# bevyengine/bevy

Measured on NVIDIA H100. Metric: entities/s propagate+cull+cluster @1M ents/256 lights, higher is better.
Workload: dtype f32

## Files before the change

bevy_b200/csrc/kernels.cu:

```cuda
#include <cstdint>
#include <cstdlib>
#include <cuda_runtime.h>

#include "device_types.cuh"
#include "kernels.cuh"

namespace b200vis {

struct Aff { float4 r0, r1, r2; };

__device__ __forceinline__ Aff affine_from_trs(float4 A, float4 q, float2 C) {
    const float sx = A.w, sy = C.x, sz = C.y;
    const float x2 = q.x + q.x, y2 = q.y + q.y, z2 = q.z + q.z;
    const float xx = q.x * x2, xy = q.x * y2, xz = q.x * z2;
    const float yy = q.y * y2, yz = q.y * z2, zz = q.z * z2;
    const float wx = q.w * x2, wy = q.w * y2, wz = q.w * z2;
    Aff a;
    a.r0 = make_float4((1.0f - (yy + zz)) * sx, (xy - wz) * sy, (xz + wy) * sz, A.x);
    a.r1 = make_float4((xy + wz) * sx, (1.0f - (xx + zz)) * sy, (yz - wx) * sz, A.y);
    a.r2 = make_float4((xz - wy) * sx, (yz + wx) * sy, (1.0f - (xx + yy)) * sz, A.z);
    return a;
}

__device__ __forceinline__ float4 affine_mul_row(float4 p, const Aff &l) {
// ... 321 lines not shown
__device__ __forceinline__ void mbar_wait_guarded(unsigned long long *bar, uint32_t parity) {
    uint32_t done = 0, spins = 0;
    while (true) {
        asm volatile("{\n.reg .pred p;\nmbarrier.try_wait.parity.shared::cta.b64 p, [%1], %2;\nselp.u32 %0, 1, 0, p;\n}\n"
                     : "=r"(done) : "r"(smem_u32(bar)), "r"(parity) : "memory");
        if (done) break;
        if (++spins > (1u << 24)) __trap();
    }
}
__device__ __forceinline__ void mbar_arrive_cta(unsigned long long *bar) {
    asm volatile("mbarrier.arrive.shared::cta.b64 _, [%0];" ::"r"(smem_u32(bar)) : "memory");
}
__device__ __forceinline__ void bulk_g2s(void *dst, const void *src, uint32_t bytes, unsigned long long *bar) {
    asm volatile("cp.async.bulk.shared::cluster.global.mbarrier::complete_tx::bytes [%0], [%1], %2, [%3];"
                 ::"r"(smem_u32(dst)), "l"(src), "r"(bytes), "r"(smem_u32(bar)) : "memory");
}
__device__ __forceinline__ void bulk_s2g(void *dst, const void *src, uint32_t bytes) {
    asm volatile("cp.async.bulk.global.shared::cta.bulk_group [%0], [%1], %2;" ::"l"(dst), "r"(smem_u32(src)), "r"(bytes) : "memory");
}

__device__ __forceinline__ void cp_async_16(void *dst, const void *src) {
    asm volatile("cp.async.cg.shared.global [%0], [%1], 16;" ::"r"(smem_u32(dst)), "l"(src) : "memory");
}
__device__ __forceinline__ void cp_async_8(void *dst, const void *src) {
    asm volatile("cp.async.ca.shared.global [%0], [%1], 8;" ::"r"(smem_u32(dst)), "l"(src) : "memory");
}
template <bool PROP, bool CULL>
__device__ __forceinline__ void issue_tile_loads(const Rows &R, const Tile &t, TileStage &S, unsigned long long *bar) {
    const uint32_t a = t.base & ~15u;
    const uint32_t cnt = ((t.base - a) + t.n_rows + 15u) & ~15u;
    uint32_t bytes = cnt * (48u + 2u);
    if (PROP) bytes += cnt * (40u + 4u);
    mbar_expect_tx(bar, bytes);
    bulk_g2s(S.gt0, R.gt0 + a, cnt * 16u, bar); bulk_g2s(S.gt1, R.gt1 + a, cnt * 16u, bar); bulk_g2s(S.gt2, R.gt2 + a, cnt * 16u, bar);
    bulk_g2s(S.flags, R.flags + a, cnt, bar); bulk_g2s(S.state, R.state + a, cnt, bar);
    if (PROP) {
        bulk_g2s(S.trsA, R.trsA + a, cnt * 16u, bar); bulk_g2s(S.trsB, R.trsB + a, cnt * 16u, bar);
        bulk_g2s(S.trsC, R.trsC + a, cnt * 8u, bar); bulk_g2s(S.topo, R.topo + a, cnt * 4u, bar);
    }
}

#ifdef B200VIS_TILE_TIMING
__device__ unsigned long long g_tile_timing[8192 * 16];
#define TT(slot) do { if (lr == 0 && blockIdx.x < 8192u) g_tile_timing[blockIdx.x * 16u + (slot)] = clock64(); } while (0)
#define TTW(slot) do { if (lr == 224u && blockIdx.x < 8192u) g_tile_timing[blockIdx.x * 16u + (slot)] = clock64(); } while (0)
__device__ unsigned long long g_tile_phase[8192 * 32];
#define TP_BEGIN() __shared__ unsigned long long tp_acc_[32]; unsigned long long tp_prev_ = clock64(); uint32_t tp_n_ = 0; \
    if (lr == 0) for (int k_ = 0; k_ < 32; ++k_) tp_acc_[k_] = 0ull
#define TP(ph) do { if (lr == 0) { const unsigned long long now_ = clock64(); \
    if ((ph) == 0) { ++tp_n_; tp_acc_[0] += 1ull; if (tp_n_ > 1u) tp_acc_[16] += 1ull; } \
    else { tp_acc_[(ph)] += now_ - tp_prev_; if (tp_n_ > 1u) tp_acc_[16 + (ph)] += now_ - tp_prev_; } \
    tp_prev_ = now_; } } while (0)
#define TP_END() do { if (lr == 0 && blockIdx.x < 8192u) for (int k_ = 0; k_ < 32; ++k_) g_tile_phase[blockIdx.x * 32u + k_] = tp_acc_[k_]; } while (0)
#else
#define TT(slot) do { } while (0)
#define TTW(slot) do { } while (0)
#define TP_BEGIN() do { } while (0)
#define TP(ph) do { } while (0)
#define TP_END() do { } while (0)
#endif
#define B200VIS_TILE_1B k_propagate_cull_tma
#define B200VIS_TILE_1B_EXT false
#include "tile_kernel_1b.cuh"
#undef B200VIS_TILE_1B
#undef B200VIS_TILE_1B_EXT
#define B200VIS_TILE_1B k_propagate_cull_tma_ext
#define B200VIS_TILE_1B_EXT true
#include "tile_kernel_1b.cuh"
#undef B200VIS_TILE_1B
#undef B200VIS_TILE_1B_EXT

template <bool WITH_TRS> struct __align__(128) LeanStage;
template <> struct __align__(128) LeanStage<true> {
    float4 gt0[kWin], gt1[kWin], gt2[kWin];
    uint32_t topo[kWin];
    uint8_t flags[kWin], state[kWin];
    float4 trsA[kWin], trsB[kWin];
    float2 trsC[kWin];
};
template <> struct __align__(128) LeanStage<false> {
    float4 gt0[kWin], gt1[kWin], gt2[kWin];
    uint32_t topo[kWin];
    uint8_t flags[kWin], state[kWin];
};
template <bool WITH_TRS>
struct LeanSmem {
    LeanStage<WITH_TRS> st[2];
    unsigned long long bar[2];
    Tile tdesc[3];
    uint32_t next_tile[2];
    float4 vplanes[kMaxViews * 5];
    float vlen[kMaxViews * 5];
    unsigned long long done[2];
    uint32_t anyflag[2];
    uint16_t parent[kTileRows];
    uint8_t pst[2][kTileRows];
    uint8_t dirty[kTileRows];
};
template <bool PROP, bool CULL, bool WITH_TRS>
__device__ __forceinline__ void issue_lean_loads(const Rows &R, const Tile &t, LeanStage<WITH_TRS> &S, unsigned long long *bar) {
    const uint32_t a = t.base & ~15u;
    const uint32_t cnt = ((t.base - a) + t.n_rows + 15u) & ~15u;
    uint32_t bytes = cnt * (48u + 2u);
    if (PROP) bytes += cnt * 4u;
    if (PROP && WITH_TRS) bytes += cnt * 40u;
    mbar_expect_tx(bar, bytes);
    bulk_g2s(S.gt0, R.gt0 + a, cnt * 16u, bar); bulk_g2s(S.gt1, R.gt1 + a, cnt * 16u, bar); bulk_g2s(S.gt2, R.gt2 + a, cnt * 16u, bar);
    bulk_g2s(S.flags, R.flags + a, cnt, bar); bulk_g2s(S.state, R.state + a, cnt, bar);
    if (PROP) bulk_g2s(S.topo, R.topo + a, cnt * 4u, bar);
    if constexpr (WITH_TRS) {
        if (PROP) {
            bulk_g2s(S.trsA, R.trsA + a, cnt * 16u, bar); bulk_g2s(S.trsB, R.trsB + a, cnt * 16u, bar);
// ... 1520 lines not shown
            uint32_t *cc = vb.chunk_count + ((size_t)parity * kMaxViews + v) * vb.chunks_stride;
            atomicOr(mask + (rnk >> 5), 1u << (rnk & 31u));
            atomicAdd(cc + ((rnk >> 5) / kChunkWords), 1u);
        }
    }
    if (SIMPLE || R.rank == nullptr) {
        if (lane < cvw.n_views && (cvw.on[lane] & 1u) && (!SIMPLE || (cvw.on[lane] & 4u))) {
            const uint32_t w0 = (row - lane) >> 5;
            if (w0 < vb.n_words) {
                vb.mask[(size_t)lane * vb.words_stride + w0] = my_ballot;
                if (my_ballot) atomicAdd(vb.chunk_count + ((size_t)parity * kMaxViews + lane) * vb.chunks_stride + (w0 / kChunkWords), __popc(my_ballot));
            }
        }
    }
    if (MERGE) {
        const bool merge = in_query && any && !(st8 & 1u);
        const uint32_t was = (st8 & S_VV_CHANGED) ? 1u : 0u;
        if (merge) R.state[row] = (uint8_t)((st8 & ~(S_VV | S_VV_CHANGED)) | 1u | (was << 1) | (was ? 0u : S_VV_CHANGED));
        const uint32_t up = __ballot_sync(0xFFFFFFFFu, merge && !was), down = __ballot_sync(0xFFFFFFFFu, merge && was);
        if (lane == 0 && up != down) atomicAdd(&stats->changed[parity][1], (uint32_t)(__popc(up) - __popc(down)));
        return;
    }
    uint32_t out = st8;
    bool vv_changed = false;
    if (in_query) {
        out = (st8 & ~(S_VV | S_VV_CHANGED)) | (any ? (1u | (prev << 1)) : 0u);
        vv_changed = (any ? 1u : 0u) != prev;
        if (vv_changed) out |= S_VV_CHANGED;
    } else {
        out = st8 & ~S_VV_CHANGED;
    }
    if (active && out != st8) R.state[row] = (uint8_t)out;
    if (R.light_snap != nullptr && (f & F_SPHERE_GT) && active) {
        const uint32_t ord = R.light_ord[row];
        if (ord < R.n_lights) R.light_snap[ord] = make_float4(g.r0.w, g.r1.w, g.r2.w, (out & 1u) ? 1.0f : 0.0f);
    }
    const uint32_t bv = __ballot_sync(0xFFFFFFFFu, vv_changed);
    if (lane == 0 && bv) atomicAdd(&stats->changed[parity][1], __popc(bv));
}

__global__ void k_mark_dirty_global(Rows R) {
    const uint32_t row = blockIdx.x * blockDim.x + threadIdx.x;
    if (row >= R.n || !(R.flags[row] & F_TCHANGED)) return;
    uint32_t c = row;
    while (true) {
        if (R.dirty[c]) break;
        R.dirty[c] = 1;
        const uint32_t p = R.parent[c];
        if (p >= R.n) break;
        c = p;
    }
}

__global__ void __launch_bounds__(kChunkWords)
k_expand_visible(VisibleBufs vb, DiffBufs db, const uint32_t *__restrict__ row_of_rank, const FrameConsts *__restrict__ fc,
                 DevStats *__restrict__ stats, uint32_t parity, uint32_t n_rows) {
    __shared__ uint32_t s_warp[32], s_diff[32];
    __shared__ uint32_t s_base, s_total;
    const uint32_t v = blockIdx.y, chunk = blockIdx.x, t = threadIdx.x;
    uint32_t *cc = vb.chunk_count + chunk_counter_index(parity, v) * vb.chunks_stride;
    const uint32_t zslot = (parity + 2u) % 3u;
    uint32_t *cc_next = vb.chunk_count + chunk_counter_index(zslot, v) * vb.chunks_stride;
    if (t == 0) cc_next[chunk] = 0;
    if (chunk == 0 && v == 0 && t < 2) stats->changed[zslot][t] = 0;
    if (v >= fc->n_views) {
        if (db.prev != nullptr && t == 0) db.chunk[(size_t)v * vb.chunks_stride + chunk] = 0;
        return;
    }
    if (!(fc->views[v].flags & 1u)) {
        if (db.prev != nullptr && t == 0) db.chunk[(size_t)v * vb.chunks_stride + chunk] = 0;
        return;
    }

    const uint32_t word = chunk * kChunkWords + t;
    uint32_t *mask = vb.mask + (size_t)v * vb.words_stride;
    uint32_t w = 0;
    if (word < vb.n_words) { w = mask[word]; if (w) mask[word] = 0; }
    const uint32_t c = __popc(w);
    if (db.prev != nullptr) {
        uint32_t a = 0, r = 0;
        if (word < vb.n_words) {
            uint32_t *pv = db.prev + (size_t)v * vb.words_stride + word;
            const uint32_t old = *pv;
            a = w & ~old; r = old & ~w;
            if (old != w) *pv = w;
            db.words[(size_t)v * vb.words_stride + word] = a;
            db.words[((size_t)gridDim.y + v) * vb.words_stride + word] = r;
        }
        uint32_t d = __popc(a) | (__popc(r) << 16);
#pragma unroll
        for (int o = 16; o > 0; o >>= 1) d += __shfl_xor_sync(0xFFFFFFFFu, d, o);
        if ((t & 31u) == 0) s_diff[t >> 5] = d;
    }
    uint32_t incl = c;
#pragma unroll
    for (int o = 1; o < 32; o <<= 1) { const uint32_t y = __shfl_up_sync(0xFFFFFFFFu, incl, o); if ((t & 31u) >= (uint32_t)o) incl += y; }
    if ((t & 31u) == 31u) s_warp[t >> 5] = incl;
    uint32_t part = 0, tot = 0;
    if (t < 32) {
        for (uint32_t i = t; i < vb.n_chunks; i += 32) { const uint32_t x = cc[i]; tot += x; if (i < chunk) part += x; }
#pragma unroll
        for (int o = 16; o > 0; o >>= 1) { part += __shfl_xor_sync(0xFFFFFFFFu, part, o); tot += __shfl_xor_sync(0xFFFFFFFFu, tot, o); }
        if (t == 0) { s_base = part; s_total = tot; }
    }
    __syncthreads();
    if (t < 32) {
        if (db.prev != nullptr) {
            uint32_t d = s_diff[t];
#pragma unroll
            for (int o = 16; o > 0; o >>= 1) d += __shfl_xor_sync(0xFFFFFFFFu, d, o);
            if (t == 0) db.chunk[(size_t)v * vb.chunks_stride + chunk] = d;
        }
        uint32_t x = s_warp[t];
#pragma unroll
        for (int o = 1; o < 32; o <<= 1) { const uint32_t y = __shfl_up_sync(0xFFFFFFFFu, x, o); if (t >= (uint32_t)o) x += y; }
        s_warp[t] = x;
    }
    __syncthreads();
    uint32_t pos = s_base + (incl - c) + ((t >> 5) ? s_warp[(t >> 5) - 1] : 0u);
    uint32_t *out = vb.lists + (size_t)v * vb.list_stride;
    uint8_t *out_cls = vb.classes ? vb.classes + (size_t)v * vb.list_stride : nullptr;
    while (w) {
        const uint32_t b = __ffs(w) - 1; w &= w - 1;
        const uint32_t rk = word * 32u + b;
        const uint32_t rw = row_of_rank ? row_of_rank[rk] : rk;
        if (out_cls) out_cls[pos] = vb.cls[rw];
        out[pos++] = rw;
    }
    if (chunk == 0 && t == 0) stats->visible_count[v] = s_total;
    (void)n_rows;
}

__global__ void __launch_bounds__(kChunkWords)
k_emit_visible_diff(VisibleBufs vb, DiffBufs db, const uint32_t *__restrict__ row_of_rank, const FrameConsts *__restrict__ fc) {
    __shared__ uint32_t s_warp[32];
    __shared__ uint32_t s_base[2], s_total[2];
    const uint32_t v = blockIdx.y, chunk = blockIdx.x, t = threadIdx.x;
    if (v >= fc->n_views || !(fc->views[v].flags & 1u)) {
        if (chunk == 0 && t < 2) db.count[v * 2 + t] = 0;
        return;
    }
    const uint32_t word = chunk * kChunkWords + t;
    uint32_t a = 0, r = 0;
    if (word < vb.n_words) {
        a = db.words[(size_t)v * vb.words_stride + word];
        r = db.words[((size_t)gridDim.y + v) * vb.words_stride + word];
    }
    const uint32_t c = __popc(a) | (__popc(r) << 16);
    uint32_t incl = c;
#pragma unroll
    for (int o = 1; o < 32; o <<= 1) { const uint32_t y = __shfl_up_sync(0xFFFFFFFFu, incl, o); if ((t & 31u) >= (uint32_t)o) incl += y; }
    if ((t & 31u) == 31u) s_warp[t >> 5] = incl;
    if (t < 32) {
        const uint32_t *cc = db.chunk + (size_t)v * vb.chunks_stride;
        uint32_t pa = 0, pr = 0, ta = 0, tr = 0;
        for (uint32_t i = t; i < vb.n_chunks; i += 32) {
            const uint32_t x = cc[i], xa = x & 0xFFFFu, xr = x >> 16;
            ta += xa; tr += xr;
            if (i < chunk) { pa += xa; pr += xr; }
        }
#pragma unroll
        for (int o = 16; o > 0; o >>= 1) {
            pa += __shfl_xor_sync(0xFFFFFFFFu, pa, o); pr += __shfl_xor_sync(0xFFFFFFFFu, pr, o);
            ta += __shfl_xor_sync(0xFFFFFFFFu, ta, o); tr += __shfl_xor_sync(0xFFFFFFFFu, tr, o);
        }
        if (t == 0) { s_base[0] = pa; s_base[1] = pr; s_total[0] = ta; s_total[1] = tr; }
    }
    __syncthreads();
    if (t < 32) {
        uint32_t x = s_warp[t];
#pragma unroll
        for (int o = 1; o < 32; o <<= 1) { const uint32_t y = __shfl_up_sync(0xFFFFFFFFu, x, o); if (t >= (uint32_t)o) x += y; }
        s_warp[t] = x;
    }
    __syncthreads();
    const uint32_t excl = (incl - c) + ((t >> 5) ? s_warp[(t >> 5) - 1] : 0u);
    uint32_t pos_a = s_base[0] + (excl & 0xFFFFu), pos_r = s_base[1] + (excl >> 16);
    uint32_t *out_a = db.lists + (size_t)v * vb.list_stride;
    uint32_t *out_r = db.lists + ((size_t)gridDim.y + v) * vb.list_stride;
    while (a) { const uint32_t b = __ffs(a) - 1; a &= a - 1; const uint32_t rk = word * 32u + b; out_a[pos_a++] = row_of_rank ? row_of_rank[rk] : rk; }
// ... 126 lines not shown
    return ((e[0] & w[0]) | (e[1] & w[1]) | (e[2] & w[2])) != 0ull;
}

template <bool EXT>
__global__ void __launch_bounds__(256)
k_cluster_assign(Rows R, Lights L, const FrameConsts *__restrict__ fc, ClusterBufs cb, DevStats *__restrict__ stats) {
    __shared__ float4 s_planes[kStagedPlanes];
    __shared__ float s_thr[kStagedPlanes];
    const uint32_t v = blockIdx.y;
    if (v >= fc->n_views) return;
    const DevClusterView &cv = fc->cviews[v];
    if (!cv.enabled) return;
    const uint32_t nx = cv.dims[0] + 1, ny_p = cv.dims[1] + 1, nz = cv.dims[2] + 1;
    const bool staged = nx + ny_p + nz <= kStagedPlanes;
    if (staged) {
        const float4 *gx = reinterpret_cast<const float4 *>(cb.blob + cv.x_off);
        const float4 *gy = reinterpret_cast<const float4 *>(cb.blob + cv.y_off);
        const float4 *gz = reinterpret_cast<const float4 *>(cb.blob + cv.z_off);
        for (uint32_t i = threadIdx.x; i < nx; i += 256) s_planes[i] = gx[i];
        for (uint32_t i = threadIdx.x; i < ny_p; i += 256) s_planes[nx + i] = gy[i];
        for (uint32_t i = threadIdx.x; i < nz; i += 256) s_planes[nx + ny_p + i] = gz[i];
        for (uint32_t i = threadIdx.x; i + 1 < cv.dims[2]; i += 256) s_thr[i] = cb.blob[cv.thr_off + i];
        __syncthreads();
    }
    const uint32_t li = blockIdx.x * 8u + (threadIdx.x >> 5), lane = threadIdx.x & 31u;
    if (li >= L.n) return;
    float px, py, pz;
    if (L.snap != nullptr) {
        const float4 sp = L.snap[li];
        if (sp.w == 0.0f) return;
        px = sp.x; py = sp.y; pz = sp.z;
    } else {
        const uint32_t row = L.row[li];
        if (!(R.state[row] & 1u)) return;
        px = R.gt0[row].w; py = R.gt1[row].w; pz = R.gt2[row].w;
    }
    const unsigned long long ll = L.layers ? L.layers[li] : 1ull;
    if (!(cv.layer_mask & ll) && !(EXT && light_layers_ext_intersect(L, fc, v, li))) return;
    const float range = L.range[li];
    ClusterTables tb;
    tb.thr = staged ? s_thr : cb.blob + cv.thr_off;
    tb.xp = staged ? s_planes : reinterpret_cast<const float4 *>(cb.blob + cv.x_off);
    tb.yp = staged ? s_planes + nx : reinterpret_cast<const float4 *>(cb.blob + cv.y_off);
    tb.zp = staged ? s_planes + nx + ny_p : reinterpret_cast<const float4 *>(cb.blob + cv.z_off);
    uint32_t *mask = cb.send + ((size_t)v * cb.words + (li >> 5)) * kMaxClusters;
    const uint32_t bit = 1u << (li & 31u);
    uint32_t count = 0;
    float this_far = 0.0f;
    if (!assign_one_light(cv, tb, px, py, pz, range, lane, this_far, count, [&](uint32_t ci) { atomicOr(mask + ci, bit); })) return;
    if (lane == 0 && this_far > 0.0f) atomicMax(cb.send + (cb.slab_words - cb.trailer) + v, __float_as_uint(this_far));
    (void)count; (void)stats;
}

constexpr uint32_t kFusedThreads = 1024;
__device__ __forceinline__ uint32_t cluster_ctarank() { uint32_t r; asm volatile("mov.u32 %0, %%cluster_ctarank;" : "=r"(r)); return r; }
__device__ __forceinline__ uint32_t cluster_nctarank() { uint32_t r; asm volatile("mov.u32 %0, %%cluster_nctarank;" : "=r"(r)); return r; }
__device__ __forceinline__ void cluster_sync_all() {
    asm volatile("barrier.cluster.arrive.release.aligned;\n\tbarrier.cluster.wait.acquire.aligned;" ::: "memory");
}
__device__ __forceinline__ uint32_t dsmem_addr(const void *p, uint32_t cta) {
    uint32_t a = (uint32_t)__cvta_generic_to_shared(p), r;
    asm volatile("mapa.shared::cluster.u32 %0, %1, %2;" : "=r"(r) : "r"(a), "r"(cta));
    return r;
}
__device__ __forceinline__ void dsmem_or(uint32_t addr, uint32_t v) {
    asm volatile("red.relaxed.cluster.shared::cluster.or.b32 [%0], %1;" ::"r"(addr), "r"(v) : "memory");
}
__device__ __forceinline__ uint32_t dsmem_ld(uint32_t addr) {
    uint32_t v; asm volatile("ld.shared::cluster.u32 %0, [%1];" : "=r"(v) : "r"(addr) : "memory"); return v;
}

__device__ __forceinline__ void st_release_sys(uint32_t *p, uint32_t v) {
    asm volatile("st.release.sys.global.u32 [%0], %1;" ::"l"(p), "r"(v) : "memory");
}
__device__ __forceinline__ uint32_t ld_acquire_sys(const uint32_t *p) {
    uint32_t v;
    asm volatile("ld.acquire.sys.global.u32 %0, [%1];" : "=r"(v) : "l"(p) : "memory");
    return v;
}
template <bool EXT>
__global__ void __launch_bounds__(kFusedThreads)
k_cluster_fused(Rows R, Lights L, const FrameConsts *__restrict__ fc, ClusterBufs cb, DevStats *__restrict__ stats) {
    extern __shared__ __align__(16) uint8_t smem_fused[];
    __shared__ float4 s_planes[kStagedPlanes];
    __shared__ float s_thr[kStagedPlanes];
    __shared__ uint32_t s_warp[32];
    __shared__ uint32_t s_total, s_far, s_base, s_farmax;
    const uint32_t v = blockIdx.y, t = threadIdx.x, lane = t & 31u, warp = t >> 5;
    const uint32_t rank = cluster_ctarank(), nrank = cluster_nctarank();
    uint32_t *offsets = cb.offsets + (size_t)v * (kMaxClusters + 1);
    if (v >= fc->n_views) return;
    const DevClusterView &cv = fc->cviews[v];
    if (!cv.enabled) {
        if (rank == 0 && t == 0) { offsets[0] = 0; stats->cl_overflow[v] = 0; stats->cl_index_count[v] = 0; stats->cl_farthest_bits[v] = 0; }
        return;
    }
    if (cb.p2p && L.per_rank) {
        if (t < cb.world) {
            const uint32_t *flag = cb.peer_flags[cb.rank] + cb.xparity * cb.world + t;
            uint32_t spins = 0;
            while ((int32_t)(ld_acquire_sys(flag) - cb.stamp) < 0) {
                __nanosleep(64);
                if (++spins > (1u << 22)) { stats->cl_overflow[v] = 2u; break; }
            }
        }
        __syncthreads();
    }
    const uint32_t nc = cv.n_clusters, per = (nc + nrank - 1) / nrank, words = (L.n + 31u) / 32u;
    uint32_t *s_mask = reinterpret_cast<uint32_t *>(smem_fused);
    for (uint32_t i = t; i < words * per; i += kFusedThreads) s_mask[i] = 0;
    if (t == 0) { s_total = 0; s_far = 0; }
    const uint32_t nx = cv.dims[0] + 1, ny_p = cv.dims[1] + 1, nz = cv.dims[2] + 1;
    const bool staged = nx + ny_p + nz <= kStagedPlanes;
    if (staged) {
        const float4 *gx = reinterpret_cast<const float4 *>(cb.blob + cv.x_off);
        const float4 *gy = reinterpret_cast<const float4 *>(cb.blob + cv.y_off);
        const float4 *gz = reinterpret_cast<const float4 *>(cb.blob + cv.z_off);
        for (uint32_t i = t; i < nx; i += kFusedThreads) s_planes[i] = gx[i];
        for (uint32_t i = t; i < ny_p; i += kFusedThreads) s_planes[nx + i] = gy[i];
        for (uint32_t i = t; i < nz; i += kFusedThreads) s_planes[nx + ny_p + i] = gz[i];
        for (uint32_t i = t; i + 1 < cv.dims[2]; i += kFusedThreads) s_thr[i] = cb.blob[cv.thr_off + i];
    }
    cluster_sync_all();
    ClusterTables tb;
    tb.thr = staged ? s_thr : cb.blob + cv.thr_off;
    tb.xp = staged ? s_planes : reinterpret_cast<const float4 *>(cb.blob + cv.x_off);
    tb.yp = staged ? s_planes + nx : reinterpret_cast<const float4 *>(cb.blob + cv.y_off);
    tb.zp = staged ? s_planes + nx + ny_p : reinterpret_cast<const float4 *>(cb.blob + cv.z_off);
    for (uint32_t li = rank + nrank * warp; li < L.n; li += nrank * (kFusedThreads / 32)) {
        float px, py, pz;
        if (L.snap != nullptr || L.per_rank) {
            const float4 sp = light_snap_of(L, li);
            if (sp.w == 0.0f) continue;
            px = sp.x; py = sp.y; pz = sp.z;
        } else {
            const uint32_t row = L.row[li];
            if (!(R.state[row] & 1u)) continue;
            px = R.gt0[row].w; py = R.gt1[row].w; pz = R.gt2[row].w;
        }
        const unsigned long long ll = light_layers_of(L, li);
        if (!(cv.layer_mask & ll) && !(EXT && light_layers_ext_intersect(L, fc, v, li))) continue;
        const uint32_t bit = 1u << (li & 31u), wbase = (li >> 5) * per;
        uint32_t count = 0;
        float this_far = 0.0f;
        const bool in = assign_one_light(cv, tb, px, py, pz, light_range_of(L, li), lane, this_far, count, [&](uint32_t ci) {
            const uint32_t owner = ci / per;
            dsmem_or(dsmem_addr(&s_mask[wbase + (ci - owner * per)], owner), bit);
        });
        if (in && lane == 0 && this_far > 0.0f) atomicMax(&s_far, __float_as_uint(this_far));
    }
    cluster_sync_all();
    const uint32_t first = rank * per, c = first + t;
    uint32_t cnt = 0;
    if (t < per && c < nc)
        for (uint32_t w = 0; w < words; ++w) cnt += __popc(s_mask[w * per + t]);
    uint32_t incl = cnt;
#pragma unroll
    for (int o = 1; o < 32; o <<= 1) { const uint32_t y = __shfl_up_sync(0xFFFFFFFFu, incl, o); if (lane >= (uint32_t)o) incl += y; }
    if (lane == 31u) s_warp[warp] = incl;
    __syncthreads();
    if (t < 32) {
        uint32_t x = s_warp[t];
#pragma unroll
        for (int o = 1; o < 32; o <<= 1) { const uint32_t y = __shfl_up_sync(0xFFFFFFFFu, x, o); if (t >= (uint32_t)o) x += y; }
        s_warp[t] = x;
        if (t == 31) s_total = x;
    }
    cluster_sync_all();
    if (t < 32) {
        uint32_t tot_r = 0, far_r = 0;
        if (t < nrank) { tot_r = dsmem_ld(dsmem_addr(&s_total, t)); far_r = dsmem_ld(dsmem_addr(&s_far, t)); }
        uint32_t b = (t < rank) ? tot_r : 0u, fm = far_r;
#pragma unroll
        for (int o = 16; o > 0; o >>= 1) {
            b += __shfl_xor_sync(0xFFFFFFFFu, b, o);
            fm = max(fm, __shfl_xor_sync(0xFFFFFFFFu, fm, o));
        }
        if (t == 0) { s_base = b; s_farmax = fm; }
    }
    asm volatile("barrier.cluster.arrive.release.aligned;" ::: "memory");
    __syncthreads();
    const uint32_t base = s_base;
    uint32_t pos = base + (incl - cnt) + (warp ? s_warp[warp - 1] : 0u);
    uint32_t *indices = cb.indices + (size_t)v * cb.index_cap;
    if (t < per && c < nc) {
        offsets[c] = pos;
        for (uint32_t w = 0; w < words; ++w) {
            uint32_t m = s_mask[w * per + t];
            while (m) {
                const uint32_t b = __ffs(m) - 1; m &= m - 1;
                if (pos < cb.index_cap) indices[pos] = w * 32u + b;
                ++pos;
            }
        }
        if (c == nc - 1) {
            offsets[nc] = pos;
            stats->cl_overflow[v] = pos > cb.index_cap ? 1u : 0u;
            stats->cl_index_count[v] = pos;
        }
    }
    if (rank == 0 && t == 0) stats->cl_farthest_bits[v] = s_farmax;
    asm volatile("barrier.cluster.wait.acquire.aligned;" ::: "memory");
}

constexpr uint32_t kListBlocks = kMaxClusters / 1024;

__global__ void __launch_bounds__(256)
k_slab_push(const FrameConsts *__restrict__ fc, ClusterBufs cb, uint32_t *__restrict__ done) {
    const uint32_t v = blockIdx.y;
    const size_t slab_words = cb.slab_words;
    if (blockIdx.x == 0 && threadIdx.x < cb.world && v < cb.trailer) {
        const size_t tr = ((size_t)cb.xparity * cb.world + cb.rank) * slab_words + (slab_words - cb.trailer) + v;
        cb.peer[threadIdx.x][tr] = cb.send[(slab_words - cb.trailer) + v];
    }
    if (v < fc->n_views && fc->cviews[v].enabled) {
// ... 1488 lines not shown
    }
    if (tile_kernel_is_tma()) {
#define B200VIS_LAUNCH_TMA(P, C, S) do { if (tile_kernel_choice() == 4) launch_tma<P, C, S, 1>(st, R, tiles, n_tiles, cvw, vb, stats, static_opt, parity, ticket, ticket_base); \
                                         else if (tile_kernel_choice() == 5 && lean_ctas_per_sm() == 4 && (P) && (C) && named_levels_only && lean_pipe()) launch_tma<P, C, S, 7>(st, R, tiles, n_tiles, cvw, vb, stats, static_opt, parity, ticket, ticket_base); \
                                         else if (tile_kernel_choice() == 5 && lean_ctas_per_sm() == 4) launch_tma<P, C, S, 4>(st, R, tiles, n_tiles, cvw, vb, stats, static_opt, parity, ticket, ticket_base); \
                                         else if (tile_kernel_choice() == 5 && lean_ctas_per_sm() == 6) launch_tma<P, C, S, 6>(st, R, tiles, n_tiles, cvw, vb, stats, static_opt, parity, ticket, ticket_base); \
                                         else if (tile_kernel_choice() == 5) launch_tma<P, C, S, 5>(st, R, tiles, n_tiles, cvw, vb, stats, static_opt, parity, ticket, ticket_base); \
                                         else launch_tma<P, C, S, 0>(st, R, tiles, n_tiles, cvw, vb, stats, static_opt, parity, ticket, ticket_base, rev); } while (0)
        if (prop && cull) { if (simple) B200VIS_LAUNCH_TMA(true, true, true); else B200VIS_LAUNCH_TMA(true, true, false); }
        else if (prop) B200VIS_LAUNCH_TMA(true, false, true);
        else if (cull) { if (simple) B200VIS_LAUNCH_TMA(false, true, true); else B200VIS_LAUNCH_TMA(false, true, false); }
#undef B200VIS_LAUNCH_TMA
        return;
    }
#define B200VIS_LAUNCH(P, C, S) ++g_launches, k_propagate_cull<P, C, S><<<n_tiles, kTileRows, 0, st>>>(R, tiles, cvw, vb, stats, static_opt, parity)
    if (prop && cull) { if (simple) B200VIS_LAUNCH(true, true, true); else B200VIS_LAUNCH(true, true, false); }
    else if (prop) B200VIS_LAUNCH(true, false, true);
    else if (cull) { if (simple) B200VIS_LAUNCH(false, true, true); else B200VIS_LAUNCH(false, true, false); }
#undef B200VIS_LAUNCH
}
void launch_propagate_cull_ext(cudaStream_t st, const Rows &R, const Tile *tiles, uint32_t n_tiles, const CullViews &cvw,
                               const VisibleBufs &vb, DevStats *stats, uint32_t stages, uint32_t static_opt, uint32_t parity,
                               uint32_t *ticket, uint32_t *ticket_base, uint32_t rev) {
    if (n_tiles == 0 || !(stages & 1u)) return;
    const bool simple = R.layers == nullptr && R.layers_ext == nullptr && R.range == nullptr && R.rank == nullptr;
    if (!(stages & 2u)) launch_tma<true, false, true, 8>(st, R, tiles, n_tiles, cvw, vb, stats, static_opt, parity, ticket, ticket_base, rev);
    else if (simple) launch_tma<true, true, true, 8>(st, R, tiles, n_tiles, cvw, vb, stats, static_opt, parity, ticket, ticket_base, rev);
    else launch_tma<true, true, false, 8>(st, R, tiles, n_tiles, cvw, vb, stats, static_opt, parity, ticket, ticket_base, rev);
}
bool tile_kernel_is_default() { return tile_kernel_choice() == 1; }
void launch_cull(cudaStream_t st, const Rows &R, const CullViews &cvw, const VisibleBufs &vb, DevStats *stats, uint32_t parity,
                 uint32_t rev) {
    if (!R.n) return;
    const bool simple = R.layers == nullptr && R.layers_ext == nullptr && R.range == nullptr && R.rank == nullptr;
    if (simple) { ++g_launches; k_cull<true, false><<<cdiv(R.n, 256), 256, 0, st>>>(R, cvw, vb, stats, parity, rev); }
    else { ++g_launches; k_cull<false, false><<<cdiv(R.n, 256), 256, 0, st>>>(R, cvw, vb, stats, parity, rev); }
}
void launch_cull_group(cudaStream_t st, const Rows &R, const CullViews &cvw, const VisibleBufs &vb, DevStats *stats, uint32_t parity,
                       uint32_t view_base, uint32_t rev) {
    if (!R.n) return;
    VisibleBufs g = vb;
    g.mask = vb.mask + (size_t)view_base * vb.words_stride;
    g.chunk_count = vb.chunk_count + chunk_counter_index(0, view_base) * vb.chunks_stride;
    const bool simple = R.layers == nullptr && R.layers_ext == nullptr && R.range == nullptr && R.rank == nullptr;
    if (simple) { ++g_launches; k_cull<true, true><<<cdiv(R.n, 256), 256, 0, st>>>(R, cvw, g, stats, parity, rev); }
    else { ++g_launches; k_cull<false, true><<<cdiv(R.n, 256), 256, 0, st>>>(R, cvw, g, stats, parity, rev); }
}
void launch_mark_dirty_global(cudaStream_t st, const Rows &R) {
    if (R.n) { ++g_launches; k_mark_dirty_global<<<cdiv(R.n, 256), 256, 0, st>>>(R); }
}
void launch_expand_visible(cudaStream_t st, const VisibleBufs &vb, const DiffBufs &db, const uint32_t *row_of_rank, const FrameConsts *fc,
                           DevStats *stats, uint32_t parity, uint32_t n_rows, uint32_t max_views) {
    if (vb.n_chunks == 0) return;
    ++g_launches; k_expand_visible<<<dim3(vb.n_chunks, max_views), kChunkWords, 0, st>>>(vb, db, row_of_rank, fc, stats, parity, n_rows);
    if (db.prev != nullptr) { ++g_launches; k_emit_visible_diff<<<dim3(vb.n_chunks, max_views), kChunkWords, 0, st>>>(vb, db, row_of_rank, fc); }
}
void launch_view_diff(cudaStream_t st, const VisibleBufs &vb, const ViewDiff &vd, const ViewSlots &vs, const uint32_t *row_of_rank,
                      const FrameConsts *fc, uint32_t parity, uint32_t slotted_views) {
    if (vb.n_chunks == 0 || slotted_views == 0) return;
    ++g_launches; k_view_diff<<<dim3(vb.n_chunks, slotted_views), kChunkWords, 0, st>>>(vb, vd, vs, row_of_rank, fc, parity);
}
void launch_emit_view_diff(cudaStream_t st, const VisibleBufs &vb, const ViewDiff &vd, const ViewSlots &vs, uint32_t n_views,
                           uint32_t slotted_views) {
    const uint32_t n_chunks = slotted_views ? vb.n_chunks : 0u;
    ++g_launches; k_view_diff_offsets<<<1, 1024, 0, st>>>(vd, vs, n_views * 8u, n_chunks, vb.chunks_stride);
    if (n_chunks == 0) return;
    ++g_launches; k_emit_view_diff<<<dim3(n_chunks, slotted_views), kChunkWords, 0, st>>>(vd, vs, vb.n_words, vb.words_stride, vb.chunks_stride);
}
void launch_publish_visible_diff(cudaStream_t st, const VisibleBufs &vb, const DiffBufs &db, uint32_t *host_rows, uint32_t host_stride,
                                 uint32_t *host_counts, uint32_t n_views, uint32_t max_views) {
    if (!n_views || db.prev == nullptr) return;
    ++g_launches; k_publish_visible_diff<<<dim3(32, n_views, 2), 256, 0, st>>>(db, vb.list_stride, host_rows, host_stride, host_counts, n_views, max_views);
}
void launch_cluster_assign(cudaStream_t st, const Rows &R, const Lights &L, const FrameConsts *fc, const ClusterBufs &cb,
                           DevStats *stats, uint32_t max_views) {
    if (L.n == 0) return;
    ++g_launches;
    if (L.layers_ext != nullptr) k_cluster_assign<true><<<dim3(cdiv(L.n, 8), max_views), 256, 0, st>>>(R, L, fc, cb, stats);
    else k_cluster_assign<false><<<dim3(cdiv(L.n, 8), max_views), 256, 0, st>>>(R, L, fc, cb, stats);
}
bool cluster_fused_fits(uint32_t n_lights) {
    const char *e = getenv("B200VIS_CLUSTER_KERNEL");
    if (e && e[0] == 's') return false;
    const size_t words = (n_lights + 31u) / 32u;
    return words * (kMaxClusters / 16) * 4 <= 200u * 1024u;
}
bool launch_cluster_fused(cudaStream_t st, const Rows &R, const Lights &L, const FrameConsts *fc, const ClusterBufs &cb,
                          DevStats *stats, uint32_t max_views) {
    static int enabled = -1, nrank_env = 0;
    static unsigned long long seen = 0;
    if (enabled < 0) {
        const char *e = getenv("B200VIS_CLUSTER_KERNEL");
        enabled = (e && e[0] == 's') ? 0 : 1;
        const char *r = getenv("B200VIS_CLUSTER_CTAS");
        nrank_env = r ? atoi(r) : 0;
    }
    if (first_call_on_device(seen)) {
        for (const void *k : {(const void *)k_cluster_fused<false>, (const void *)k_cluster_fused<true>}) {
            cudaFuncSetAttribute(k, cudaFuncAttributeMaxDynamicSharedMemorySize, 200 * 1024);
            cudaFuncSetAttribute(k, cudaFuncAttributeNonPortableClusterSizeAllowed, 1);
        }
    }
    const bool ext = L.layers_ext != nullptr;
    if (!enabled) return false;
    const uint32_t words = (L.n + 31u) / 32u;
    static_assert(kMaxClusters / 4 <= kFusedThreads, "a CTA of the fused cluster kernel owns more clusters than it has threads");
    uint32_t nrank = (nrank_env == 4 || nrank_env == 8 || nrank_env == 16) ? (uint32_t)nrank_env : 8u;
    size_t smem = (size_t)words * (kMaxClusters / nrank) * 4;
    if (smem > 200u * 1024u) { nrank = 16; smem = (size_t)words * (kMaxClusters / nrank) * 4; }
    if (smem > 200u * 1024u) return false;
    cudaLaunchConfig_t cfg = {};
    cfg.gridDim = dim3(nrank, max_views); cfg.blockDim = dim3(kFusedThreads); cfg.dynamicSmemBytes = smem; cfg.stream = st;
    cudaLaunchAttribute attr[1];
    attr[0].id = cudaLaunchAttributeClusterDimension;
    attr[0].val.clusterDim.x = nrank; attr[0].val.clusterDim.y = 1; attr[0].val.clusterDim.z = 1;
    cfg.attrs = attr; cfg.numAttrs = 1;
    static int schedulable[2][17] = {};
    int &sched = schedulable[ext ? 1 : 0][nrank];
    if (sched == 0) {
        cudaLaunchConfig_t probe = cfg;
        probe.dynamicSmemBytes = 200u * 1024u;
        int n_clusters = 0;
        const cudaError_t e = ext ? cudaOccupancyMaxActiveClusters(&n_clusters, k_cluster_fused<true>, &probe)
                                  : cudaOccupancyMaxActiveClusters(&n_clusters, k_cluster_fused<false>, &probe);
        sched = (e == cudaSuccess && n_clusters > 0) ? 1 : -1;
        if (e != cudaSuccess) (void)cudaGetLastError();
    }
    if (sched < 0) return false;
    ++g_launches;
    const cudaError_t le = ext ? cudaLaunchKernelEx(&cfg, k_cluster_fused<true>, R, L, fc, cb, stats)
                               : cudaLaunchKernelEx(&cfg, k_cluster_fused<false>, R, L, fc, cb, stats);
    if (le == cudaSuccess) return true;
    (void)cudaGetLastError();
    return false;
}
void launch_publish_visible(cudaStream_t st, const VisibleBufs &vb, const DevStats *stats, uint32_t *host_rows, uint32_t host_stride,
                            uint32_t n_rows, uint32_t n_views, uint8_t *host_classes) {
    if (!n_views || !n_rows) return;
    static int sms = 0;
    if (!sms) { int dev = 0; cudaGetDevice(&dev); cudaDeviceGetAttribute(&sms, cudaDevAttrMultiProcessorCount, dev); if (sms <= 0) sms = 132; }
    ++g_launches; k_publish_visible<<<dim3(min(cdiv(n_rows, 256), 2u * (uint32_t)sms), n_views), 256, 0, st>>>(vb.lists, vb.list_stride, stats, host_rows, host_stride, n_views, vb.classes, host_classes);
}
void launch_publish_clusters(cudaStream_t st, const FrameConsts *fc, const ClusterBufs &cb, uint32_t *host_offsets, uint32_t *host_indices,
                             uint32_t host_cap, const DevStats *stats, uint32_t *host_stats, uint32_t changed_slot, uint32_t frame, uint32_t max_views,
                             uint32_t *host_view_stats) {
    ++g_launches; k_publish_clusters<<<dim3(kMaxClusters / 256 + 1, max_views), 256, 0, st>>>(fc, cb.offsets, cb.indices, cb.index_cap, host_offsets, host_indices,
                                                                                host_cap, stats, host_stats, changed_slot, frame, host_view_stats);
}
void launch_shadow_cull(cudaStream_t st, const Rows &R, const ShadowBufs &sb, const uint32_t *view_sets, uint32_t n_views,
                        uint32_t n_words, uint32_t n_chunks, uint32_t words_stride, uint32_t chunks_stride, DevStats *stats, uint32_t changed_slot,
                        const ShadowSink &sink, const ShadowDiff &sd) {
    const bool diff = sd.added != nullptr;
    if (!sb.n_lights || (!R.n && sink.entities == nullptr && !diff)) return;
    ++g_launches; k_shadow_select<<<cdiv(sb.n_lights, 128), 128, 0, st>>>(sb, R.rank, view_sets, words_stride, n_views);
    if (!R.n) {
        if (sink.entities != nullptr) { ++g_launches; k_shadow_offsets<<<1, 1024, 0, st>>>(sb, 0u, chunks_stride, sink.dev_offsets, sink.offsets, sink.active); }
        if (diff) { ++g_launches; k_shadow_diff_offsets<<<1, 1024, 0, st>>>(sb, sd, 0u, chunks_stride); }
        return;
    }
    ++g_launches;
    if (sb.layers_ext != nullptr) k_shadow_cull<true><<<cdiv(R.n, 256), 256, 0, st>>>(R, sb, words_stride, chunks_stride, stats, changed_slot);
    else k_shadow_cull<false><<<cdiv(R.n, 256), 256, 0, st>>>(R, sb, words_stride, chunks_stride, stats, changed_slot);
    const dim3 grid(n_chunks, sb.n_lights);
    if (sink.entities != nullptr) { ++g_launches; k_shadow_offsets<<<1, 1024, 0, st>>>(sb, n_chunks, chunks_stride, sink.dev_offsets, sink.offsets, sink.active); }
    ++g_launches;
// ... 274 lines not shown
        const uint32_t r = (uint32_t)(i / k), j = (uint32_t)(i - (size_t)r * k);
        const bool keep = r < p.n_new;
        const size_t s = keep ? (size_t)p.new_to_old[r] * k + j : 0;
        switch (c.elem) {
        case 1: static_cast<uint8_t *>(c.dst)[i] = keep ? static_cast<const uint8_t *>(c.src)[s] : (uint8_t)c.fill; break;
        case 4: static_cast<uint32_t *>(c.dst)[i] = keep ? static_cast<const uint32_t *>(c.src)[s] : (uint32_t)c.fill; break;
        case 8: static_cast<unsigned long long *>(c.dst)[i] = keep ? static_cast<const unsigned long long *>(c.src)[s] : c.fill; break;
        default: static_cast<uint4 *>(c.dst)[i] = keep ? static_cast<const uint4 *>(c.src)[s] : make_uint4(0u, 0u, 0u, 0u); break;
        }
    }
}
static uint32_t list_grid(uint32_t max_count) { return std::max<uint32_t>(1u, std::min<uint32_t>(cdiv(max_count, 256), 1024u)); }
void launch_mark_listed_rows(cudaStream_t st, const RowLists &L, uint32_t max_count, uint8_t *mark, uint32_t n_rows) {
    if (!L.n_lists || !max_count) return;
    ++g_launches; k_mark_listed_rows<<<dim3(list_grid(max_count), L.n_lists), 256, 0, st>>>(L, mark, n_rows);
}
void launch_mark_set_rows(cudaStream_t st, const uint32_t *sets, uint32_t stride, uint32_t n_sets, uint32_t n_words,
                          const uint32_t *row_of_rank, uint8_t *mark) {
    if (!n_sets || !n_words) return;
    ++g_launches; k_mark_set_rows<<<dim3(cdiv(n_words, 256), n_sets), 256, 0, st>>>(sets, stride, n_words, row_of_rank, mark);
}
void launch_renumber_listed_rows(cudaStream_t st, const RowLists &L, uint32_t max_count, const uint32_t *old_to_new, uint32_t n_old) {
    if (!L.n_lists || !max_count) return;
    ++g_launches; k_renumber_listed_rows<<<dim3(list_grid(max_count), L.n_lists), 256, 0, st>>>(L, old_to_new, n_old);
}
void launch_gather_u32(cudaStream_t st, const uint32_t *src, const uint32_t *idx, uint32_t n, uint32_t *dst) {
    if (n) { ++g_launches; k_gather_u32<<<cdiv(n, 256), 256, 0, st>>>(src, idx, n, dst); }
}
void launch_compact_ranks(cudaStream_t st, const uint32_t *old_row_of_rank, const uint64_t *old_keys, uint32_t n_old, const uint32_t *dropped,
                          uint32_t n_drop, const uint32_t *old_to_new, uint32_t *row_of_rank, uint32_t *rank, uint64_t *keys,
                          uint32_t *src_rank, uint32_t *not_identity) {
    if (n_old) { ++g_launches; k_compact_ranks<<<cdiv(n_old, 256), 256, 0, st>>>(old_row_of_rank, old_keys, n_old, dropped, n_drop, old_to_new,
                                                                                  row_of_rank, rank, keys, src_rank, not_identity); }
}
void launch_permute_rows(cudaStream_t st, const RowPermute &p) {
    if (!p.n_cols || !p.n_old) return;
    uint32_t k = 1;
    for (uint32_t c = 0; c < p.n_cols; ++c) k = std::max(k, p.col[c].per_row);
    const uint32_t blocks = (uint32_t)std::min<size_t>(((size_t)p.n_old * k + 255) / 256, 8192);
    ++g_launches; k_permute_rows<<<dim3(blocks, p.n_cols), 256, 0, st>>>(p);
}

}

#ifdef B200VIS_TILE_TIMING
extern "C" __attribute__((visibility("default"))) int b200vis_debug_tile_timing(unsigned long long *out, unsigned n_ctas) {
    if (n_ctas > 8192u) n_ctas = 8192u;
    return (int)cudaMemcpyFromSymbol(out, b200vis::g_tile_timing, (size_t)n_ctas * 16 * sizeof(unsigned long long));
}
extern "C" __attribute__((visibility("default"))) int b200vis_debug_tile_phases(unsigned long long *out, unsigned n_ctas) {
    if (n_ctas > 8192u) n_ctas = 8192u;
    return (int)cudaMemcpyFromSymbol(out, b200vis::g_tile_phase, (size_t)n_ctas * 32 * sizeof(unsigned long long));
}
#endif
```

bevy_b200/csrc/tile_kernel_1b.cuh:

```cuda
template <bool PROP, bool CULL, bool SIMPLE>
__global__ void __launch_bounds__(kTileRows, 4)
B200VIS_TILE_1B(Rows R, const Tile *__restrict__ tiles, uint32_t n_tiles, const __grid_constant__ CullViews cvw,
                VisibleBufs vb, DevStats *__restrict__ stats, uint32_t static_opt, uint32_t parity,
                uint32_t *__restrict__ ticket, uint32_t ticket_base, uint32_t rev) {
    constexpr bool EXT = B200VIS_TILE_1B_EXT;
    extern __shared__ __align__(128) uint8_t smem_raw[];
    TmaSmem &s = *reinterpret_cast<TmaSmem *>(smem_raw);
    const uint32_t lr = threadIdx.x;
    if (lr == 0) {
        mbar_init(&s.bar[0], 1); mbar_init(&s.bar[1], 1);
        asm volatile("fence.mbarrier_init.release.cluster;" ::: "memory");
    }
    __syncthreads();
    TP_BEGIN();
    asm volatile("griddepcontrol.wait;" ::: "memory");
    auto tile_at = [&](uint32_t i) -> const Tile & { return tiles[rev ? n_tiles - 1u - i : i]; };
    uint32_t t = blockIdx.x;
    if (lr == 0 && t < n_tiles) issue_tile_loads<PROP, CULL>(R, tile_at(t), s.st[0], &s.bar[0]);
    uint32_t n_gt_total = 0, n_vv_total = 0;
    for (uint32_t it = 0; t < n_tiles; ++it) {
        TP(0);
        const uint32_t sidx = it & 1u;
        const Tile tile = tile_at(t);
        TP(1);
        mbar_wait(&s.bar[sidx], (it >> 1) & 1u);
        TP(2);
        TileStage &S = s.st[sidx];
        const uint32_t off = tile.base & 15u;
        const uint32_t li = off + lr;
        const bool active = lr < tile.n_rows;
        const uint32_t row = tile.base + lr;
        const uint32_t f = active ? S.flags[li] : 0u;
        const uint32_t st8 = active ? S.state[li] : 0u;
        float4 bA = make_float4(0, 0, 0, 0); float2 bB = make_float2(0, 0);
        if (!PROP && CULL && active) { bA = R.bndA[row]; bB = R.bndB[row]; }

        bool visited = false, changed = false;
        const bool ext_mark = EXT && (st8 & S_GT_EXT);
        if (PROP) {
            const uint32_t topo = active ? S.topo[li] : T_DETACHED;
            const uint32_t depth = (topo >> 9) & 0x1FFu, plocal = topo & 0x1FFu;
            const bool tchanged = f & F_TCHANGED;
            const bool has_children = topo & T_HAS_CHILDREN;
            bool dirty = tchanged;
            if (static_opt && R.dirty != nullptr) {
                dirty = active && R.dirty[row];
            } else if (static_opt && tile.n_levels > 1 && __syncthreads_or(tchanged && depth > 0)) {
                s.parent[lr] = (uint16_t)((depth > 0) ? plocal : 0xFFFFu);
                s.dirty[lr] = 0;
                __syncthreads();
                if (active && tchanged) {
                    uint32_t c = lr;
                    while (!s.dirty[c]) {
                        s.dirty[c] = 1;
                        const uint32_t p = s.parent[c];
                        if (p == 0xFFFFu) break;
                        c = p;
                    }
                }
                __syncthreads();
                dirty = s.dirty[lr];
            }
            TP(3);
            const Aff l = affine_from_trs(S.trsA[li], S.trsB[li], S.trsC[li]);
            if (CULL && active) { cp_async_16(&S.trsA[li], R.bndA + row); cp_async_8(&S.trsC[li], R.bndB + row); }
            const uint32_t my_level = (active && !(topo & T_DETACHED)) ? depth : 0xFFFFFFFFu;
            if (active && (topo & T_DETACHED) && has_children) s.pst[lr] = 0;
            if (my_level == 0) {
// ... 217 lines not shown
```

Measured before the change: 13.33 billion.

## Restructure visible-list expansion to warp-per-word scatter and size fused cluster CTAs

The expand kernel now runs with fewer threads per block, each handling several mask words. It builds a shared list of nonzero words with their output offsets, then has each warp expand one word per iteration with lanes mapped to bits. This replaces the serial per-thread bit loop with coalesced row_of_rank lookups and output writes, which should reduce divergence on dense masks. The fused cluster kernel now launches only as many threads as clusters per CTA instead of a fixed 1024, and debug-only probe timing scopes are added.

Measured after the change: 14.12 billion (median of 6 runs). +5.9%, better.

```diff
diff --git a/bevy_b200/csrc/kernels.cu b/bevy_b200/csrc/kernels.cu
--- a/bevy_b200/csrc/kernels.cu
+++ b/bevy_b200/csrc/kernels.cu
@@ -397,12 +397,28 @@
     else { tp_acc_[(ph)] += now_ - tp_prev_; if (tp_n_ > 1u) tp_acc_[16 + (ph)] += now_ - tp_prev_; } \
     tp_prev_ = now_; } } while (0)
 #define TP_END() do { if (lr == 0 && blockIdx.x < 8192u) for (int k_ = 0; k_ < 32; ++k_) g_tile_phase[blockIdx.x * 32u + k_] = tp_acc_[k_]; } while (0)
+struct ProbeRec { unsigned long long t0, t1; uint32_t kind, tag, blk, threads; };
+constexpr uint32_t kProbeCap = 1u << 18;
+__device__ ProbeRec g_probe[kProbeCap];
+__device__ uint32_t g_probe_n;
+__device__ __forceinline__ unsigned long long global_ns() { unsigned long long t; asm volatile("mov.u64 %0, %%globaltimer;" : "=l"(t)); return t; }
+struct ProbeScope {
+    unsigned long long t0; uint32_t kind, tag; bool on;
+    __device__ ProbeScope(uint32_t k, uint32_t tg) : t0(0), kind(k), tag(tg), on(threadIdx.x == 0) { if (on) t0 = global_ns(); }
+    __device__ ~ProbeScope() {
+        if (!on) return;
+        const uint32_t i = atomicAdd(&g_probe_n, 1u);
+        if (i < kProbeCap) g_probe[i] = ProbeRec{t0, global_ns(), kind, tag, blockIdx.x + (blockIdx.y << 16), blockDim.x};
+    }
+};
+#define PROBE_SCOPE(kind, tag) ProbeScope probe_scope_((kind), (tag))
 #else
 #define TT(slot) do { } while (0)
 #define TTW(slot) do { } while (0)
 #define TP_BEGIN() do { } while (0)
 #define TP(ph) do { } while (0)
 #define TP_END() do { } while (0)
+#define PROBE_SCOPE(kind, tag) do { } while (0)
 #endif
 #define B200VIS_TILE_1B k_propagate_cull_tma
 #define B200VIS_TILE_1B_EXT false
@@ -2029,12 +2045,17 @@
     }
 }
 
-__global__ void __launch_bounds__(kChunkWords)
+constexpr uint32_t kExpandThreads = 256, kExpandWords = kChunkWords / kExpandThreads, kExpandBatch = 8;
+__global__ void __launch_bounds__(kExpandThreads, 4)
 k_expand_visible(VisibleBufs vb, DiffBufs db, const uint32_t *__restrict__ row_of_rank, const FrameConsts *__restrict__ fc,
                  DevStats *__restrict__ stats, uint32_t parity, uint32_t n_rows) {
-    __shared__ uint32_t s_warp[32], s_diff[32];
-    __shared__ uint32_t s_base, s_total;
-    const uint32_t v = blockIdx.y, chunk = blockIdx.x, t = threadIdx.x;
+    constexpr uint32_t kWarps = kExpandThreads / 32;
+    __shared__ uint32_t s_warp[kWarps], s_diff[kWarps];
+    __shared__ uint32_t s_base, s_total, s_nnz;
+    __shared__ uint32_t s_w[kChunkWords];
+    __shared__ uint32_t s_nz_word[kChunkWords], s_nz_pos[kChunkWords];
+    PROBE_SCOPE(1u, 0u);
+    const uint32_t v = blockIdx.y, chunk = blockIdx.x, t = threadIdx.x, lane = t & 31u, warp = t >> 5;
     uint32_t *cc = vb.chunk_count + chunk_counter_index(parity, v) * vb.chunks_stride;
     const uint32_t zslot = (parity + 2u) % 3u;
     uint32_t *cc_next = vb.chunk_count + chunk_counter_index(zslot, v) * vb.chunks_stride;
@@ -2049,30 +2070,38 @@
         return;
     }
 
-    const uint32_t word = chunk * kChunkWords + t;
+    const uint32_t word0 = chunk * kChunkWords;
     uint32_t *mask = vb.mask + (size_t)v * vb.words_stride;
-    uint32_t w = 0;
-    if (word < vb.n_words) { w = mask[word]; if (w) mask[word] = 0; }
-    const uint32_t c = __popc(w);
-    if (db.prev != nullptr) {
-        uint32_t a = 0, r = 0;
-        if (word < vb.n_words) {
+    uint32_t d = 0;
+#pragma unroll
+    for (uint32_t k = 0; k < kExpandWords; ++k) {
+        const uint32_t lw = k * kExpandThreads + t, word = word0 + lw;
+        uint32_t w = 0;
+        if (word < vb.n_words) { w = mask[word]; if (w) mask[word] = 0; }
+        s_w[lw] = w;
+        if (db.prev != nullptr && word < vb.n_words) {
             uint32_t *pv = db.prev + (size_t)v * vb.words_stride + word;
             const uint32_t old = *pv;
-            a = w & ~old; r = old & ~w;
+            const uint32_t a = w & ~old, r = old & ~w;
             if (old != w) *pv = w;
             db.words[(size_t)v * vb.words_stride + word] = a;
             db.words[((size_t)gridDim.y + v) * vb.words_stride + word] = r;
-        }
-        uint32_t d = __popc(a) | (__popc(r) << 16);
+            d += __popc(a) | (__popc(r) << 16);
+        }
+    }
+    if (db.prev != nullptr) {
 #pragma unroll
         for (int o = 16; o > 0; o >>= 1) d += __shfl_xor_sync(0xFFFFFFFFu, d, o);
-        if ((t & 31u) == 0) s_diff[t >> 5] = d;
-    }
+        if (lane == 0) s_diff[warp] = d;
+    }
+    __syncthreads();
+    uint32_t mine[kExpandWords], c = 0;
+#pragma unroll
+    for (uint32_t k = 0; k < kExpandWords; ++k) { mine[k] = s_w[t * kExpandWords + k]; c += __popc(mine[k]) | (mine[k] ? 0x10000u : 0u); }
     uint32_t incl = c;
 #pragma unroll
-    for (int o = 1; o < 32; o <<= 1) { const uint32_t y = __shfl_up_sync(0xFFFFFFFFu, incl, o); if ((t & 31u) >= (uint32_t)o) incl += y; }
-    if ((t & 31u) == 31u) s_warp[t >> 5] = incl;
+    for (int o = 1; o < 32; o <<= 1) { const uint32_t y = __shfl_up_sync(0xFFFFFFFFu, incl, o); if (lane >= (uint32_t)o) incl += y; }
+    if (lane == 31u) s_warp[warp] = incl;
     uint32_t part = 0, tot = 0;
     if (t < 32) {
         for (uint32_t i = t; i < vb.n_chunks; i += 32) { const uint32_t x = cc[i]; tot += x; if (i < chunk) part += x; }
@@ -2083,26 +2112,50 @@
     __syncthreads();
     if (t < 32) {
         if (db.prev != nullptr) {
-            uint32_t d = s_diff[t];
-#pragma unroll
-            for (int o = 16; o > 0; o >>= 1) d += __shfl_xor_sync(0xFFFFFFFFu, d, o);
-            if (t == 0) db.chunk[(size_t)v * vb.chunks_stride + chunk] = d;
-        }
-        uint32_t x = s_warp[t];
+            uint32_t dd = t < kWarps ? s_diff[t] : 0u;
+#pragma unroll
+            for (int o = 16; o > 0; o >>= 1) dd += __shfl_xor_sync(0xFFFFFFFFu, dd, o);
+            if (t == 0) db.chunk[(size_t)v * vb.chunks_stride + chunk] = dd;
+        }
+        uint32_t x = t < kWarps ? s_warp[t] : 0u;
 #pragma unroll
         for (int o = 1; o < 32; o <<= 1) { const uint32_t y = __shfl_up_sync(0xFFFFFFFFu, x, o); if (t >= (uint32_t)o) x += y; }
-        s_warp[t] = x;
+        if (t < kWarps) s_warp[t] = x;
+        if (t == 31) s_nnz = x >> 16;
     }
     __syncthreads();
-    uint32_t pos = s_base + (incl - c) + ((t >> 5) ? s_warp[(t >> 5) - 1] : 0u);
+    uint32_t ex = (incl - c) + (warp ? s_warp[warp - 1] : 0u);
+    uint32_t pos = ex & 0xFFFFu, nz = ex >> 16;
+#pragma unroll
+    for (uint32_t k = 0; k < kExpandWords; ++k) {
+        if (mine[k]) { s_nz_word[nz] = t * kExpandWords + k; s_nz_pos[nz] = pos; ++nz; }
+        pos += __popc(mine[k]);
+    }
+    __syncthreads();
+    const uint32_t nnz = s_nnz, base = s_base, below = (1u << lane) - 1u;
     uint32_t *out = vb.lists + (size_t)v * vb.list_stride;
     uint8_t *out_cls = vb.classes ? vb.classes + (size_t)v * vb.list_stride : nullptr;
-    while (w) {
-        const uint32_t b = __ffs(w) - 1; w &= w - 1;
-        const uint32_t rk = word * 32u + b;
-        const uint32_t rw = row_of_rank ? row_of_rank[rk] : rk;
-        if (out_cls) out_cls[pos] = vb.cls[rw];
-        out[pos++] = rw;
+    for (uint32_t b0 = warp * kExpandBatch; b0 < nnz; b0 += kWarps * kExpandBatch) {
+        uint32_t wv[kExpandBatch], rw[kExpandBatch], cl[kExpandBatch];
+#pragma unroll
+        for (uint32_t k = 0; k < kExpandBatch; ++k) {
+            const uint32_t i = b0 + k;
+            const uint32_t lw = i < nnz ? s_nz_word[i] : 0u;
+            wv[k] = i < nnz ? s_w[lw] : 0u;
+            const uint32_t rk = (word0 + lw) * 32u + lane;
+            rw[k] = ((wv[k] >> lane) & 1u) ? (row_of_rank ? row_of_rank[rk] : rk) : 0u;
+        }
+        if (out_cls) {
+#pragma unroll
+            for (uint32_t k = 0; k < kExpandBatch; ++k) cl[k] = ((wv[k] >> lane) & 1u) ? vb.cls[rw[k]] : 0u;
+        }
+#pragma unroll
+        for (uint32_t k = 0; k < kExpandBatch; ++k) {
+            if (!((wv[k] >> lane) & 1u)) continue;
+            const uint32_t p = base + s_nz_pos[b0 + k] + __popc(wv[k] & below);
+            if (out_cls) out_cls[p] = (uint8_t)cl[k];
+            out[p] = rw[k];
+        }
     }
     if (chunk == 0 && t == 0) stats->visible_count[v] = s_total;
     (void)n_rows;
@@ -2335,7 +2388,7 @@
     (void)count; (void)stats;
 }
 
-constexpr uint32_t kFusedThreads = 1024;
+constexpr uint32_t kFusedMaxThreads = kMaxClusters / 4;
 __device__ __forceinline__ uint32_t cluster_ctarank() { uint32_t r; asm volatile("mov.u32 %0, %%cluster_ctarank;" : "=r"(r)); return r; }
 __device__ __forceinline__ uint32_t cluster_nctarank() { uint32_t r; asm volatile("mov.u32 %0, %%cluster_nctarank;" : "=r"(r)); return r; }
 __device__ __forceinline__ void cluster_sync_all() {
@@ -2362,14 +2415,15 @@
     return v;
 }
 template <bool EXT>
-__global__ void __launch_bounds__(kFusedThreads)
+__global__ void __launch_bounds__(kFusedMaxThreads)
 k_cluster_fused(Rows R, Lights L, const FrameConsts *__restrict__ fc, ClusterBufs cb, DevStats *__restrict__ stats) {
     extern __shared__ __align__(16) uint8_t smem_fused[];
     __shared__ float4 s_planes[kStagedPlanes];
     __shared__ float s_thr[kStagedPlanes];
     __shared__ uint32_t s_warp[32];
     __shared__ uint32_t s_total, s_far, s_base, s_farmax;
-    const uint32_t v = blockIdx.y, t = threadIdx.x, lane = t & 31u, warp = t >> 5;
+    PROBE_SCOPE(2u, 0u);
+    const uint32_t v = blockIdx.y, t = threadIdx.x, lane = t & 31u, warp = t >> 5, nthr = blockDim.x;
     const uint32_t rank = cluster_ctarank(), nrank = cluster_nctarank();
     uint32_t *offsets = cb.offsets + (size_t)v * (kMaxClusters + 1);
     if (v >= fc->n_views) return;
@@ -2391,7 +2445,7 @@
     }
     const uint32_t nc = cv.n_clusters, per = (nc + nrank - 1) / nrank, words = (L.n + 31u) / 32u;
     uint32_t *s_mask = reinterpret_cast<uint32_t *>(smem_fused);
-    for (uint32_t i = t; i < words * per; i += kFusedThreads) s_mask[i] = 0;
+    for (uint32_t i = t; i < words * per; i += nthr) s_mask[i] = 0;
     if (t == 0) { s_total = 0; s_far = 0; }
     const uint32_t nx = cv.dims[0] + 1, ny_p = cv.dims[1] + 1, nz = cv.dims[2] + 1;
     const bool staged = nx + ny_p + nz <= kStagedPlanes;
@@ -2399,10 +2453,10 @@
         const float4 *gx = reinterpret_cast<const float4 *>(cb.blob + cv.x_off);
         const float4 *gy = reinterpret_cast<const float4 *>(cb.blob + cv.y_off);
         const float4 *gz = reinterpret_cast<const float4 *>(cb.blob + cv.z_off);
-        for (uint32_t i = t; i < nx; i += kFusedThreads) s_planes[i] = gx[i];
-        for (uint32_t i = t; i < ny_p; i += kFusedThreads) s_planes[nx + i] = gy[i];
-        for (uint32_t i = t; i < nz; i += kFusedThreads) s_planes[nx + ny_p + i] = gz[i];
-        for (uint32_t i = t; i + 1 < cv.dims[2]; i += kFusedThreads) s_thr[i] = cb.blob[cv.thr_off + i];
+        for (uint32_t i = t; i < nx; i += nthr) s_planes[i] = gx[i];
+        for (uint32_t i = t; i < ny_p; i += nthr) s_planes[nx + i] = gy[i];
+        for (uint32_t i = t; i < nz; i += nthr) s_planes[nx + ny_p + i] = gz[i];
+        for (uint32_t i = t; i + 1 < cv.dims[2]; i += nthr) s_thr[i] = cb.blob[cv.thr_off + i];
     }
     cluster_sync_all();
     ClusterTables tb;
@@ -2410,7 +2464,7 @@
     tb.xp = staged ? s_planes : reinterpret_cast<const float4 *>(cb.blob + cv.x_off);
     tb.yp = staged ? s_planes + nx : reinterpret_cast<const float4 *>(cb.blob + cv.y_off);
     tb.zp = staged ? s_planes + nx + ny_p : reinterpret_cast<const float4 *>(cb.blob + cv.z_off);
-    for (uint32_t li = rank + nrank * warp; li < L.n; li += nrank * (kFusedThreads / 32)) {
+    for (uint32_t li = rank + nrank * warp; li < L.n; li += nrank * (nthr / 32u)) {
         float px, py, pz;
         if (L.snap != nullptr || L.per_rank) {
             const float4 sp = light_snap_of(L, li);
@@ -2443,7 +2497,7 @@
     if (lane == 31u) s_warp[warp] = incl;
     __syncthreads();
     if (t < 32) {
-        uint32_t x = s_warp[t];
+        uint32_t x = t < nthr / 32u ? s_warp[t] : 0u;
 #pragma unroll
         for (int o = 1; o < 32; o <<= 1) { const uint32_t y = __shfl_up_sync(0xFFFFFFFFu, x, o); if (t >= (uint32_t)o) x += y; }
         s_warp[t] = x;
@@ -4038,7 +4092,7 @@
 void launch_expand_visible(cudaStream_t st, const VisibleBufs &vb, const DiffBufs &db, const uint32_t *row_of_rank, const FrameConsts *fc,
                            DevStats *stats, uint32_t parity, uint32_t n_rows, uint32_t max_views) {
     if (vb.n_chunks == 0) return;
-    ++g_launches; k_expand_visible<<<dim3(vb.n_chunks, max_views), kChunkWords, 0, st>>>(vb, db, row_of_rank, fc, stats, parity, n_rows);
+    ++g_launches; k_expand_visible<<<dim3(vb.n_chunks, max_views), kExpandThreads, 0, st>>>(vb, db, row_of_rank, fc, stats, parity, n_rows);
     if (db.prev != nullptr) { ++g_launches; k_emit_visible_diff<<<dim3(vb.n_chunks, max_views), kChunkWords, 0, st>>>(vb, db, row_of_rank, fc); }
 }
 void launch_view_diff(cudaStream_t st, const VisibleBufs &vb, const ViewDiff &vd, const ViewSlots &vs, const uint32_t *row_of_rank,
@@ -4090,13 +4144,12 @@
     const bool ext = L.layers_ext != nullptr;
     if (!enabled) return false;
     const uint32_t words = (L.n + 31u) / 32u;
-    static_assert(kMaxClusters / 4 <= kFusedThreads, "a CTA of the fused cluster kernel owns more clusters than it has threads");
     uint32_t nrank = (nrank_env == 4 || nrank_env == 8 || nrank_env == 16) ? (uint32_t)nrank_env : 8u;
     size_t smem = (size_t)words * (kMaxClusters / nrank) * 4;
     if (smem > 200u * 1024u) { nrank = 16; smem = (size_t)words * (kMaxClusters / nrank) * 4; }
     if (smem > 200u * 1024u) return false;
     cudaLaunchConfig_t cfg = {};
-    cfg.gridDim = dim3(nrank, max_views); cfg.blockDim = dim3(kFusedThreads); cfg.dynamicSmemBytes = smem; cfg.stream = st;
+    cfg.gridDim = dim3(nrank, max_views); cfg.blockDim = dim3(kMaxClusters / nrank); cfg.dynamicSmemBytes = smem; cfg.stream = st;
     cudaLaunchAttribute attr[1];
     attr[0].id = cudaLaunchAttributeClusterDimension;
     attr[0].val.clusterDim.x = nrank; attr[0].val.clusterDim.y = 1; attr[0].val.clusterDim.z = 1;
@@ -4477,4 +4530,13 @@
     if (n_ctas > 8192u) n_ctas = 8192u;
     return (int)cudaMemcpyFromSymbol(out, b200vis::g_tile_phase, (size_t)n_ctas * 32 * sizeof(unsigned long long));
 }
+extern "C" __attribute__((visibility("default"))) long long b200vis_debug_probe(void *out, unsigned cap) {
+    uint32_t n = 0;
+    cudaError_t e = cudaMemcpyFromSymbol(&n, b200vis::g_probe_n, sizeof n);
+    const uint32_t k = std::min(std::min(n, cap), b200vis::kProbeCap);
+    if (e == cudaSuccess && k) e = cudaMemcpyFromSymbol(out, b200vis::g_probe, (size_t)k * sizeof(b200vis::ProbeRec));
+    const uint32_t zero = 0;
+    if (e == cudaSuccess) e = cudaMemcpyToSymbol(b200vis::g_probe_n, &zero, sizeof zero);
+    return e == cudaSuccess ? (long long)n : -(long long)e;
+}
 #endif
diff --git a/bevy_b200/csrc/tile_kernel_1b.cuh b/bevy_b200/csrc/tile_kernel_1b.cuh
--- a/bevy_b200/csrc/tile_kernel_1b.cuh
+++ b/bevy_b200/csrc/tile_kernel_1b.cuh
@@ -14,6 +14,7 @@
     __syncthreads();
     TP_BEGIN();
     asm volatile("griddepcontrol.wait;" ::: "memory");
+    PROBE_SCOPE(0u, ticket_base);
     auto tile_at = [&](uint32_t i) -> const Tile & { return tiles[rev ? n_tiles - 1u - i : i]; };
     uint32_t t = blockIdx.x;
     if (lr == 0 && t < n_tiles) issue_tile_loads<PROP, CULL>(R, tile_at(t), s.st[0], &s.bar[0]);
```
